# ashispati/ar-vae

Measured on AMD Instinct MI355X. Metric: training images/sec (dSprites beta-VAE+AR, per-GPU batch 512), higher is better.
Workload: dtype f32 (conv MFMAs: scaled 2-term fp16 split, 3 products, fp32-accurate)

## Files before the change

### ar-vae_amd/csrc/conv32.h

```cpp
#pragma once
#include "common.h"
#include "reduce.h"
#include "midprep.h"
#include "regloss.h"

namespace arvae {

bool conv32_fits(const arvae_link_t *l);
int conv32_down(const arvae_link_t *l, const Operand &hi, const float *bias, int relu, const float *gate, const uint16_t *gate_bits,
                uint16_t *bits_out, float *out, hipStream_t s, const float *wprep, const unsigned *amax_in, unsigned *amax_out);
int conv32_up(const arvae_link_t *l, const Operand &lo, const float *bias, int relu, const float *gate, const uint16_t *gate_bits,
              uint16_t *bits_out, float *out, hipStream_t s, const float *wprep, const unsigned *amax_in, unsigned *amax_out);
bool conv32_down_chain_fits(const arvae_link_t *a, const arvae_link_t *b);
int conv32_down_chain(const arvae_link_t *a, const arvae_link_t *b, const float *hi, const unsigned *amax_in, const float *bias_a,
                      uint16_t *bits_a, float *out_a, const float *wprep_a, unsigned *amax_a, const float *bias_b, uint16_t *bits_b,
                      float *out_b, const float *wprep_b, unsigned *amax_b, hipStream_t s);
bool conv32_up_reg_fits(const arvae_link_t *l);
int conv32_up_reg(const arvae_link_t *l, const Operand &lo, const float *bias, uint16_t *bits_out, float *out, const float *wprep,
                  const unsigned *amax_in, unsigned *amax_out, const RegArgs &reg, int r, hipStream_t s);

int64_t conv32_prep_floats();
int64_t conv32_scratch_floats();
int conv32_weight_prep(const float *const *wts, float *const *preps, int n_layers, hipStream_t s);
int conv32_weight_prep_with_mid(const float *const *wts, float *const *preps, int n_layers, const MidPrepArgs &mid, hipStream_t s);
int conv32_amax(const float *x, int64_t count, unsigned *out, hipStream_t s);

int64_t conv32_wgrad_ws_floats(const arvae_link_t *l);
int conv32_wgrad(const arvae_link_t *l, const Operand &lo, const Operand &hi, float *dwt, float *dbias, int bias_mode,
                 float *slab, hipStream_t s, const unsigned *amax_lo, const unsigned *amax_hi);
int conv32_wgrad_partial(const arvae_link_t *l, const Operand &lo, const Operand &hi, float *dwt, float *dbias, int bias_mode,
                         float *slab, hipStream_t s, SlabJob *job, const unsigned *amax_lo, const unsigned *amax_hi);
bool conv32_pair_fits(const arvae_link_t *l, bool up, const float *gate, const uint16_t *gate_bits, int bias_mode);
bool conv32_pair_c1_fits(const arvae_link_t *l, bool up, const uint16_t *gate_bits);
int conv32_pair(const arvae_link_t *l, bool up, const float *g, const float *x_in, const float *gate, const uint16_t *gate_bits,
                float *d_in, const float *wprep, float *dwt, float *dbias, float *slab, hipStream_t s, SlabJob *job,
                const unsigned *amax_g, const unsigned *amax_x, unsigned *amax_out, const float *c1_img, float *c1_slab, SlabJob *c1_job);

}
```

### ar-vae_amd/csrc/conv32.hip

```cpp
#include <mutex>
#include "diag.h"
#include "common.h"
#include "conv32_common.h"
#include "conv32.h"
#include "reduce.h"
#include "midprep.h"
#include "prep32.h"
#include "regloss.h"
#include "down32p.h"
#include "wgrad32r.h"

#include <type_traits>

namespace arvae {

template <int LO, int STRIDE, int PX = 128>
struct PatchLoader {
    using T = Tile<LO, PX>;
    static constexpr int SZ = STRIDE * LO;
    static constexpr int PR = STRIDE * T::TR + 2, PC = STRIDE * T::TC + 2;
    static constexpr int SLOTS = T::TI * PR * PC * 8;
    static constexpr int ITERS = (SLOTS + 255) / 256;
    float4 r[ITERS];
    unsigned rel[ITERS];
// ... 922 lines not shown
            out[16 * C32 * C32 + threadIdx.x] = tot;
        }
    }
}
template <int LO, int BIAS>
__global__ __launch_bounds__(256, 1) void wgrad32x_kernel(const float *__restrict__ lo, const float *__restrict__ hi,
                                                          float *__restrict__ slab, int n_img, int n_tiles, const unsigned *amax_lo,
                                                          const unsigned *amax_hi) {
    wgrad32x_body<LO, BIAS>(lo, hi, slab, n_img, n_tiles, amax_lo, amax_hi, blockIdx.x, gridDim.x);
}

template <int MODE, int BIAS>
__global__ __launch_bounds__(256, 1) void pair4_down_kernel(const float *__restrict__ g_hi, Ep32 ep,
                                                           const float *__restrict__ w_lo, const float *__restrict__ w_hi,
                                                           float *__restrict__ slab, int n_img, int tiles_a, int tiles_b, int grid_a,
                                                           const unsigned *amax_lo, const unsigned *amax_hi) {
    if ((int)blockIdx.x < grid_a) down32s_body<4, MODE>(g_hi, ep, n_img, tiles_a, blockIdx.x, grid_a);
    else wgrad32x_body<4, BIAS>(w_lo, w_hi, slab, n_img, tiles_b, amax_lo, amax_hi, blockIdx.x - grid_a, gridDim.x - grid_a);
}
template <int MODE, int BIAS>
__global__ __launch_bounds__(256, 1) void pair4_up_kernel(const float *__restrict__ g_lo, Ep32 ep,
                                                         const float *__restrict__ w_lo, const float *__restrict__ w_hi,
                                                         float *__restrict__ slab, int n_img, int tiles_a, int tiles_b, int grid_a,
                                                         const unsigned *amax_lo, const unsigned *amax_hi) {
    if ((int)blockIdx.x < grid_a) up32x_body<4, MODE, 32>(g_lo, ep, n_img, tiles_a, blockIdx.x, grid_a);
    else wgrad32x_body<4, BIAS>(w_lo, w_hi, slab, n_img, tiles_b, amax_lo, amax_hi, blockIdx.x - grid_a, gridDim.x - grid_a);
}


template <int LO, int MODE, int BIAS>
__global__ __launch_bounds__(512) __attribute__((amdgpu_waves_per_eu(2, 2))) void pair_down_wgrad_kernel(
    const float *__restrict__ g_hi, Ep32 ep, int n_img, int tiles_a, int grid_a, const float *__restrict__ w_lo, const float *__restrict__ w_hi,
    float *__restrict__ slab, int total_steps, int steps_per_wg, const unsigned *amax_lo, const unsigned *amax_hi) {
    if ((int)blockIdx.x < grid_a) down32p_body<LO, MODE>(g_hi, ep, n_img, tiles_a, blockIdx.x, grid_a);
    else wgrad32r_body<LO, BIAS>(w_lo, w_hi, slab, n_img, total_steps, steps_per_wg, amax_lo, amax_hi, blockIdx.x - grid_a);
}
template <int MODE, int BIAS, bool C1W = false>
__global__ __launch_bounds__(512) __attribute__((amdgpu_waves_per_eu(2, 2))) void pair_up16_wgrad_kernel(
    const float *__restrict__ g_lo, Ep32 ep, int n_img, int tiles_a, int grid_a, const float *__restrict__ w_lo, const float *__restrict__ w_hi,
    float *__restrict__ slab, int total_steps, int steps_per_wg, const unsigned *amax_lo, const unsigned *amax_hi, C1Wgrad c1) {
    if ((int)blockIdx.x < grid_a) up32p_body<MODE, C1W>(g_lo, ep, n_img, tiles_a, blockIdx.x, grid_a, c1);
    else wgrad32r_body<16, BIAS>(w_lo, w_hi, slab, n_img, total_steps, steps_per_wg, amax_lo, amax_hi, blockIdx.x - grid_a);
}
template <int MODE, int BIAS>
__global__ __launch_bounds__(512) __attribute__((amdgpu_waves_per_eu(2, 2))) void pair_up8_wgrad_kernel(
    const float *__restrict__ g_lo, Ep32 ep, int n_img, int tiles_a, int grid_a, const float *__restrict__ w_lo, const float *__restrict__ w_hi,
    float *__restrict__ slab, int total_steps, int steps_per_wg, const unsigned *amax_lo, const unsigned *amax_hi) {
    if ((int)blockIdx.x < grid_a) {
        if (threadIdx.x >= 256) return;
        up32x_body<8, MODE, 32>(g_lo, ep, n_img, tiles_a, blockIdx.x, grid_a);
    } else wgrad32r_body<8, BIAS>(w_lo, w_hi, slab, n_img, total_steps, steps_per_wg, amax_lo, amax_hi, blockIdx.x - grid_a);
}

static int cu_count() { return device_cu_count(); }

template <int LO, int PX = 128> static constexpr int tiles_for(int n) {
    using T = Tile<LO, PX>;
    return T::TI == 1 ? n * (LO / T::TR) : (n + T::TI - 1) / T::TI;
}
static int grid_for_tiles(int tiles) {
    const int cap = cu_count() < AMAX_N / 4 ? cu_count() : AMAX_N / 4;
    return tiles < cap ? tiles : cap;
}

bool conv32_fits(const arvae_link_t *l) {
    return l->chi == 32 && l->clo == 32 && l->kh == 4 && l->kw == 4 && l->stride == 2 && l->pad == 1 &&
           l->hh == l->hw && l->lh == l->lw && (l->lh == 16 || l->lh == 8 || l->lh == 4) && l->hi_perm_c == 0 &&
           l->lo_perm_c == 0 && (int64_t)l->n * l->hh * l->hw * PIXB < (1ll << 31) - (1ll << 20);
}

template <class K> static void allow_lds(K kernel, int bytes) {
    (void)hipFuncSetAttribute((const void *)kernel, hipFuncAttributeMaxDynamicSharedMemorySize, bytes);
}

template <int A, int B> struct MaxOf { static constexpr int value = A > B ? A : B; };

constexpr int LDS_DOWN_S = (PatchLoader<4, 2, 32>::BUF2_DW + 4 * 16 * 64) * 4;
static int down_small_grid(int tiles) {
    int g = tiles < 2 * cu_count() ? tiles : 2 * cu_count();
    return g < AMAX_N ? g : AMAX_N;
}

template <int MODE> static void launch_down_small(const Operand &hi, const Ep32 &ep, int n, hipStream_t s) {
    const int tiles = tiles_for<4, 32>(n);
    static std::once_flag attr;
    std::call_once(attr, [&] { allow_lds(down32s_kernel<4, MODE>, LDS_DOWN_S); });
    ARVAE_LAUNCH((down32s_kernel<4, MODE>), dim3(down_small_grid(tiles)), dim3(256), LDS_DOWN_S, s, hi.v, ep, n, tiles);
}
template <int LO, int MODE, int PX>
static void launch_up_px(const Operand &lo, const Ep32 &ep, int n, hipStream_t s) {
    const int tiles = tiles_for<LO, PX>(n), grid = grid_for_tiles(tiles);
    if constexpr (LO == 16 && PX == 128 && MODE != EP_GATE_F) {
        constexpr int LDSP = (2 * 2 * PatchLoader<16, 1, 128>::PLANE_DW) * 4 + 4 * 4 * 4 * 64 * 16;
        static std::once_flag attrp;
        std::call_once(attrp, [&] { allow_lds(up32p_kernel<MODE>, LDSP); });
        ARVAE_LAUNCH((up32p_kernel<MODE>), dim3(grid), dim3(512), LDSP, s, lo.v, ep, n, tiles);
    } else {
        constexpr int LDSX = 2 * PatchLoader<LO, 1, PX>::PLANE_DW * 4;
        static std::once_flag attrx;
        std::call_once(attrx, [&] { allow_lds(up32x_kernel<LO, MODE, PX>, LDSX); });
        ARVAE_LAUNCH((up32x_kernel<LO, MODE, PX>), dim3(grid), dim3(256), LDSX, s, lo.v, ep, n, tiles);
    }
}
template <int LO, int MODE>
static void launch_up_v(const Operand &lo, const Ep32 &ep, int n, hipStream_t s) {
    if (LO == 4 && 2 * tiles_for<LO, 128>(n) <= cu_count()) launch_up_px<4, MODE, 32>(lo, ep, n, s);
// ... 186 lines not shown
        allow_lds(wgrad32r_kernel<LO, 2>, LDS);
    });
    if (bias_mode == 1) ARVAE_LAUNCH((wgrad32r_kernel<LO, 1>), dim3(grid), dim3(512), LDS, s, lo, hi, slab, l->n, total, spw, amax_lo, amax_hi);
    else if (bias_mode == 2) ARVAE_LAUNCH((wgrad32r_kernel<LO, 2>), dim3(grid), dim3(512), LDS, s, lo, hi, slab, l->n, total, spw, amax_lo, amax_hi);
    else ARVAE_LAUNCH((wgrad32r_kernel<LO, 0>), dim3(grid), dim3(512), LDS, s, lo, hi, slab, l->n, total, spw, amax_lo, amax_hi);
    return check_launch(LO == 16 ? "wgrad32_kernel<16>" : "wgrad32_kernel<8>");
}
static int conv32_wgrad_stream(const arvae_link_t *l, const Operand &lo, const Operand &hi, float *slab, int bias_mode, const unsigned *amax_lo,
                               const unsigned *amax_hi, hipStream_t s) {
    return l->lh == 16 ? launch_stream<16>(l, lo.v, hi.v, slab, bias_mode, amax_lo, amax_hi, s)
                       : launch_stream<8>(l, lo.v, hi.v, slab, bias_mode, amax_lo, amax_hi, s);
}

static int conv32_wgrad_groups(const arvae_link_t *l) {
    if (conv32_wgrad_stream_fits(l)) return conv32_wgrad_stream_groups(l);
    return grid_for_tiles(tiles_for<4, 64>(l->n));
}

int64_t conv32_wgrad_ws_floats(const arvae_link_t *l) {
    return (int64_t)conv32_wgrad_groups(l) * WG32_SLAB;
}

constexpr int LDS_WGRAD_X4 = 2 * (PatchLoader<4, 2, 64>::PLANE_DW / PSB * WGRAD_PSB_H + 64 * WGRAD_PSB_L) * 4;
static int launch_wgrad_x4(const arvae_link_t *l, const Operand &lo, const Operand &hi, float *slab, int bias_mode, int grid,
                           const unsigned *amax_lo, const unsigned *amax_hi, hipStream_t s) {
    const int tiles = tiles_for<4, 64>(l->n);
    static std::once_flag attr;
    std::call_once(attr, [&] {
        allow_lds(wgrad32x_kernel<4, 0>, LDS_WGRAD_X4);
        allow_lds(wgrad32x_kernel<4, 1>, LDS_WGRAD_X4);
        allow_lds(wgrad32x_kernel<4, 2>, LDS_WGRAD_X4);
    });
    if (bias_mode == 1)
        ARVAE_LAUNCH((wgrad32x_kernel<4, 1>), dim3(grid), dim3(256), LDS_WGRAD_X4, s, lo.v, hi.v, slab, l->n, tiles, amax_lo, amax_hi);
    else if (bias_mode == 2)
        ARVAE_LAUNCH((wgrad32x_kernel<4, 2>), dim3(grid), dim3(256), LDS_WGRAD_X4, s, lo.v, hi.v, slab, l->n, tiles, amax_lo, amax_hi);
    else
        ARVAE_LAUNCH((wgrad32x_kernel<4, 0>), dim3(grid), dim3(256), LDS_WGRAD_X4, s, lo.v, hi.v, slab, l->n, tiles, amax_lo, amax_hi);
    return check_launch("wgrad32_kernel<4>");
}

int conv32_wgrad_partial(const arvae_link_t *l, const Operand &lo, const Operand &hi, float *dwt, float *dbias, int bias_mode,
                         float *slab, hipStream_t s, SlabJob *job, const unsigned *amax_lo, const unsigned *amax_hi) {
    ARVAE_REQUIRE(amax_lo != nullptr && amax_hi != nullptr, "conv32_wgrad: the operands' maxima are needed");
    const int grid = conv32_wgrad_groups(l);
    const int rc = conv32_wgrad_stream_fits(l) ? conv32_wgrad_stream(l, lo, hi, slab, bias_mode, amax_lo, amax_hi, s)
                                               : launch_wgrad_x4(l, lo, hi, slab, bias_mode, grid, amax_lo, amax_hi, s);
    *job = SlabJob{slab, dwt, bias_mode ? dbias : nullptr, grid, SLAB_C32, bias_mode};
    return rc;
}

constexpr int PAIR_SPLIT_C1_PERCENT = 62;
constexpr int PAIR_SPLIT_PERCENT = 50;
bool conv32_pair_fits(const arvae_link_t *l, bool up, const float *gate, const uint16_t *gate_bits, int bias_mode) {
    static const bool off4 = diag_env("ARVAE_NO_PAIR4") != nullptr;
    static const bool off = diag_env("ARVAE_NO_PAIR32") != nullptr;
    if ((gate == nullptr && gate_bits == nullptr) || bias_mode != (up ? 2 : 1)) return false;
    if (l->lh == 4) {
        const int wg_tiles = tiles_for<4, 64>(l->n), dg_tiles = tiles_for<4, 32>(l->n);
        return !off4 && wg_tiles >= 8 && wg_tiles + (dg_tiles + 1) / 2 <= cu_count() && conv32_wgrad_groups(l) == wg_tiles;
    }
    if (off || gate_bits == nullptr || !conv32_wgrad_stream_fits(l)) return false;
    if (l->n * (l->lh * l->lh / 32) < 4 * cu_count()) return false;
    if (!up && l->lh == 8 && tiles_for<8, 128>(l->n) > cu_count()) return false;
    return true;
}

template <int LO> static int launch_pair_big(const arvae_link_t *l, bool up, const float *g, const float *x_in, const Ep32 &ep, float *slab,
                                             const unsigned *amax_g, const unsigned *amax_x, hipStream_t s, int *grid_b_out,
                                             const C1Wgrad *c1 = nullptr, int *grid_a_out = nullptr) {
    const int cus = cu_count() < AMAX_N / 4 ? cu_count() : AMAX_N / 4;
    int grid_a = cus * (c1 != nullptr ? PAIR_SPLIT_C1_PERCENT : PAIR_SPLIT_PERCENT) / 100;
    if (grid_a < 1) grid_a = 1;
    const int tiles_a = up ? l->n * DownK<LO>::TILES_PER_IMG : (LO == 16 ? tiles_for<16, 128>(l->n) : tiles_for<8, 32>(l->n));
    {
        const int run = (tiles_a + grid_a - 1) / grid_a;
        grid_a = (tiles_a + run - 1) / run;
    }
    if (grid_a_out != nullptr) *grid_a_out = grid_a;
    ARVAE_REQUIRE(c1 == nullptr || grid_a <= 256, "pair_up16_wgrad: %d workgroups of the Up half exceed the first layer's 256 weight-gradient slabs", grid_a);
    int total, spw, grid_b;
    stream_geometry(l, cus - grid_a, total, spw, grid_b);
    *grid_b_out = grid_b;
    constexpr int LDS_W = RowStream<LO>::LDS_DW * 4;
    const dim3 grid(grid_a + grid_b);
    if (up) {
        constexpr int LDS = MaxOf<LDS_W, DownK<LO>::LDS_DW * 4>::value;
        static std::once_flag attr;
        std::call_once(attr, [&] { allow_lds(pair_down_wgrad_kernel<LO, EP_GATE_B, 2>, LDS); });
        ARVAE_LAUNCH((pair_down_wgrad_kernel<LO, EP_GATE_B, 2>), grid, dim3(512), LDS, s, g, ep, l->n, tiles_a, grid_a, x_in, g, slab, total, spw,
                     amax_x, amax_g);
        return check_launch(LO == 16 ? "pair(down32<16> + wgrad32<16>)" : "pair(down32<8> + wgrad32<8>)");
    }
    if constexpr (LO == 16) {
        constexpr int LDS_U = (2 * 2 * PatchLoader<16, 1, 128>::PLANE_DW) * 4 + 4 * 4 * 4 * 64 * 16;
        constexpr int LDS = MaxOf<LDS_W, LDS_U>::value;
        static std::once_flag attr;
        if (c1 != nullptr) {
            constexpr int LDS_C = MaxOf<LDS_W, LDS_U + 4 * C1W_WAVE_DW * 4>::value;
            static std::once_flag attr_c;
            std::call_once(attr_c, [&] { allow_lds(pair_up16_wgrad_kernel<EP_GATE_B, 1, true>, LDS_C); });
            ARVAE_LAUNCH((pair_up16_wgrad_kernel<EP_GATE_B, 1, true>), grid, dim3(512), LDS_C, s, g, ep, l->n, tiles_a, grid_a, g, x_in,
                         slab, total, spw, amax_g, amax_x, *c1);
            return check_launch("pair(up32<16> + wgrad32<16> + wgrad_c1)");
        }
        std::call_once(attr, [&] { allow_lds(pair_up16_wgrad_kernel<EP_GATE_B, 1>, LDS); });
        ARVAE_LAUNCH((pair_up16_wgrad_kernel<EP_GATE_B, 1>), grid, dim3(512), LDS, s, g, ep, l->n, tiles_a, grid_a, g, x_in, slab,
                     total, spw, amax_g, amax_x, C1Wgrad{nullptr, nullptr});
        return check_launch("pair(up32<16> + wgrad32<16>)");
    } else {
        constexpr int LDS = MaxOf<LDS_W, 2 * PatchLoader<8, 1, 32>::PLANE_DW * 4>::value;
        static std::once_flag attr;
        std::call_once(attr, [&] { allow_lds(pair_up8_wgrad_kernel<EP_GATE_B, 1>, LDS); });
        ARVAE_LAUNCH((pair_up8_wgrad_kernel<EP_GATE_B, 1>), grid, dim3(512), LDS, s, g, ep, l->n, tiles_a, grid_a, g, x_in, slab, total,
                     spw, amax_g, amax_x);
        return check_launch("pair(up32<8> + wgrad32<8>)");
    }
}

bool conv32_pair_c1_fits(const arvae_link_t *l, bool up, const uint16_t *gate_bits) {
    return !up && l->lh == 16 && gate_bits != nullptr;
}
int conv32_pair(const arvae_link_t *l, bool up, const float *g, const float *x_in, const float *gate, const uint16_t *gate_bits,
                float *d_in, const float *wprep, float *dwt, float *dbias, float *slab, hipStream_t s, SlabJob *job,
                const unsigned *amax_g, const unsigned *amax_x, unsigned *amax_out, const float *c1_img, float *c1_slab, SlabJob *c1_job) {
    ARVAE_REQUIRE(wprep != nullptr && amax_g != nullptr && amax_x != nullptr, "conv32_pair: prepared weights and the operands' maxima are needed");
    Ep32 ep{nullptr, gate_bits ? nullptr : gate, gate_bits, nullptr, d_in, reinterpret_cast<const uint4 *>(wprep), amax_g, amax_out};
    if (l->lh != 4) {
        int grid_b = 0, grid_a = 0;
        C1Wgrad c1{c1_img, c1_slab};
        const bool fuse = c1_img != nullptr && c1_slab != nullptr && c1_job != nullptr && conv32_pair_c1_fits(l, up, gate_bits);
        ARVAE_REQUIRE(fuse || c1_img == nullptr, "conv32_pair: this layer cannot carry the first layer's weight gradient");
        const int rc = l->lh == 16 ? launch_pair_big<16>(l, up, g, x_in, ep, slab, amax_g, amax_x, s, &grid_b, fuse ? &c1 : nullptr, &grid_a)
                                   : launch_pair_big<8>(l, up, g, x_in, ep, slab, amax_g, amax_x, s, &grid_b);
        *job = SlabJob{slab, dwt, dbias, grid_b, SLAB_C32, up ? 2 : 1};
        if (fuse) *c1_job = SlabJob{c1_slab, nullptr, nullptr, grid_a, SLAB_C1, 1};
        return rc;
    }
    constexpr int LDS_U = 2 * PatchLoader<4, 1, 32>::PLANE_DW * 4;
    constexpr int LDS = MaxOf<LDS_WGRAD_X4, MaxOf<LDS_DOWN_S, LDS_U>::value>::value;
    const int wg_tiles = tiles_for<4, 64>(l->n), dg_tiles = tiles_for<4, 32>(l->n), grid_a = (dg_tiles + 1) / 2;
    static std::once_flag attr;
    std::call_once(attr, [&] {
        allow_lds(pair4_down_kernel<EP_GATE_F, 2>, LDS);
        allow_lds(pair4_down_kernel<EP_GATE_B, 2>, LDS);
        allow_lds(pair4_up_kernel<EP_GATE_F, 1>, LDS);
        allow_lds(pair4_up_kernel<EP_GATE_B, 1>, LDS);
    });
    const dim3 grid(grid_a + wg_tiles);
    if (up) {
        if (gate_bits) ARVAE_LAUNCH((pair4_down_kernel<EP_GATE_B, 2>), grid, dim3(256), LDS, s, g, ep, x_in, g, slab, l->n, dg_tiles, wg_tiles, grid_a, amax_x, amax_g);
        else ARVAE_LAUNCH((pair4_down_kernel<EP_GATE_F, 2>), grid, dim3(256), LDS, s, g, ep, x_in, g, slab, l->n, dg_tiles, wg_tiles, grid_a, amax_x, amax_g);
    } else {
        if (gate_bits) ARVAE_LAUNCH((pair4_up_kernel<EP_GATE_B, 1>), grid, dim3(256), LDS, s, g, ep, g, x_in, slab, l->n, dg_tiles, wg_tiles, grid_a, amax_g, amax_x);
        else ARVAE_LAUNCH((pair4_up_kernel<EP_GATE_F, 1>), grid, dim3(256), LDS, s, g, ep, g, x_in, slab, l->n, dg_tiles, wg_tiles, grid_a, amax_g, amax_x);
    }
    *job = SlabJob{slab, dwt, dbias, wg_tiles, SLAB_C32, up ? 2 : 1};
    return check_launch(up ? "pair4(down32 + wgrad32)" : "pair4(up32 + wgrad32)");
}

int conv32_wgrad(const arvae_link_t *l, const Operand &lo, const Operand &hi, float *dwt, float *dbias, int bias_mode,
                 float *slab, hipStream_t s, const unsigned *amax_lo, const unsigned *amax_hi) {
    SlabJob job;
    if (int rc = conv32_wgrad_partial(l, lo, hi, dwt, dbias, bias_mode, slab, s, &job, amax_lo, amax_hi)) return rc;
    return slab_reduce(job, s);
}

}

#ifdef ARVAE_STAMPS
extern "C" int arvae_debug_stamps(unsigned long long *out, int count) {
    return (int)hipMemcpyFromSymbol(out, HIP_SYMBOL(arvae::g_stamps), sizeof(unsigned long long) * count);
}
#endif
#ifdef D32K_STAMPS
extern "C" int arvae_debug_d32k_stamps(unsigned long long *out, int count) {
    return (int)hipMemcpyFromSymbol(out, HIP_SYMBOL(arvae::g_d32k_stamps), sizeof(unsigned long long) * count);
}
#endif
#ifdef WGR_STAMPS
extern "C" int arvae_debug_wgr_stamps(unsigned long long *out, int count) {
    return (int)hipMemcpyFromSymbol(out, HIP_SYMBOL(arvae::g_wgr_stamps), sizeof(unsigned long long) * count);
}
#endif
```

### ar-vae_amd/csrc/plan.hip

```cpp
#include "diag.h"
#include "common.h"
#include "dense.h"
#include "reduce.h"
#include "midprep.h"
#include "regloss.h"
#include "vae_finish.h"
#include "amax.h"
#include "conv32.h"
#include "conv_c1.h"
#include "conv64.h"
#include "link.h"
#include "heads.h"
#include "midblock.h"
#include "losses.h"

namespace arvae {

__global__ __launch_bounds__(256) void latent_bwd_full_kernel(const float *__restrict__ g_z, const float *__restrict__ dz_reg,
                                                               const float *__restrict__ dz_extra, const float *__restrict__ mu,
                                                               const float *__restrict__ sigma, const float *__restrict__ eps,
                                                               const float *__restrict__ g_loss, const float *__restrict__ kl,
                                                               const float *__restrict__ cap, float beta, float inv_batch,
                                                               float reg_scale, int64_t count, float *__restrict__ d_mu,
                                                               float *__restrict__ d_ls) {
// ... 214 lines not shown
                if (int rc = conv32_amax(a.in, in_elems(l, a.n), a.tmp_amax, hs)) return rc;
                in_amax = a.tmp_amax;
            }
            return l.is_up ? conv32_up(&lk, make_operand(&op), b, 1, nullptr, nullptr, a.bits_out, a.out, hs, a.wprep, in_amax, a.out_amax)
                           : conv32_down(&lk, make_operand(&op), b, 1, nullptr, nullptr, a.bits_out, a.out, hs, a.wprep, in_amax, a.out_amax);
        }
        return conv_c1_down(&lk, make_operand(&op), w, b, 1, nullptr, nullptr, a.bits_out, a.out, hs, a.out_amax);
    }
    if (conv64_fits(&lk, l.is_up != 0) && a.tmp_amax != nullptr && wide_stack(&lk)) {
        hipStream_t hs = as_stream(a.st);
        if (in_amax == nullptr && conv64s_fits(&lk, l.is_up != 0)) {
            if (int rc = conv32_amax(a.in, in_elems(l, a.n), a.tmp_amax, hs)) return rc;
            in_amax = a.tmp_amax;
        }
        a.out_has = a.out_amax != nullptr;
        return l.is_up ? conv64_up(&lk, make_operand(&op), w, b, l.act, a.mask, a.out, a.link_ws, hs, nullptr, in_amax, a.out_amax, a.wide_prep)
                       : conv64_down(&lk, make_operand(&op), w, b, l.act, a.mask, a.out, a.link_ws, hs, nullptr, in_amax, a.out_amax, a.wide_prep);
    }
    if (!l.is_up && a.out_amax != nullptr && wide_stack(&lk) && !conv64_fits(&lk, false) && single_channel_down_fits(&lk)) {
        a.out_has = true;
        return single_channel_down(&lk, make_operand(&op), w, b, l.act, a.mask, a.out, as_stream(a.st), a.out_amax);
    }
    return l.is_up ? arvae_link_up(&lk, &op, w, b, l.act, a.mask, a.out, a.link_ws, a.st)
                   : arvae_link_down(&lk, &op, w, b, l.act, a.mask, a.out, a.link_ws, a.st);
}

struct LayerBwd {
    const arvae_layer_t *l;
    int32_t n;
    const float *params;
    float *grads;
    const float *in, *out;
    const uint8_t *mask;
    const float *g;
    bool g_is_pre;
    const float *g_scale;
    const float *gate;
    const uint16_t *gate_bits;
    const GateOp *gate_op;
    GateOp gate_store;
    float *d_in;
    float *slab, *link_ws, *own_slab;
    DenseWgradBatch *defer;
    SlabReduceBatch *rdefer;
    arvae_stream_t st;
    const float *wprep;
    float *wide_prep;
    const unsigned *g_amax, *in_amax;
    unsigned *tmp_amax, *tmp2_amax, *din_amax;
    const float *c1_img;
    float *c1_slab;
    SlabJob *c1_job;
    const VaeFinishArgs *finish;
    bool gated;
    bool din_has;
    bool finish_taken;
};

static int layer_backward(LayerBwd &a) {
    const arvae_layer_t &l = *a.l;
    const int32_t n = a.n;
    const arvae_link_t lk = with_batch(l, n);
    const arvae_stream_t st = a.st;
    const float *const g = a.g, *const in = a.in, *const gate = a.gate;
    const uint16_t *const gate_bits = a.gate_bits;
    float *const d_in = a.d_in;
    const unsigned *g_amax = a.g_amax, *in_amax = a.in_amax;
    a.gated = a.din_has = a.finish_taken = false;
    const bool c32 = conv32_fits(&lk) && a.wprep != nullptr && a.tmp_amax != nullptr && a.tmp2_amax != nullptr;
    auto need_g = [&]() -> int {
        if (g_amax != nullptr) return ARVAE_OK;
        g_amax = a.tmp_amax;
        return conv32_amax(g, out_elems(l, n), a.tmp_amax, as_stream(st));
    };
    auto need_in = [&]() -> int {
        if (in_amax != nullptr) return ARVAE_OK;
        in_amax = a.tmp2_amax;
        return conv32_amax(in, in_elems(l, n), a.tmp2_amax, as_stream(st));
    };
    arvae_operand_t gop = a.g_is_pre ? plain(g) : arvae_operand_t{g, a.out, a.mask, l.act};
    if (!a.g_is_pre && (a.mask != nullptr || l.act != ARVAE_ACT_NONE) && (conv64_fits(&lk, false) || conv64_fits(&lk, true))) {
        if (int rc = arvae_operand_apply(&gop, out_elems(l, n), const_cast<float *>(g), st)) return rc;
        gop = plain(g);
        g_amax = nullptr;
    }
    const arvae_operand_t xin = plain(in);
    const float *w = a.params + l.w_off;
    float *dw = a.grads + l.w_off, *db = bias_of(l, a.grads);
    const int bias_mode = db ? (l.is_up ? 2 : 1) : 0;
    hipStream_t hs = as_stream(st);
    const bool own_slab_free = a.rdefer != nullptr && a.own_slab != nullptr && a.rdefer->count < SLAB_BATCH_MAX;
    if (d_in != nullptr && own_slab_free && gop.y == nullptr && a.g_scale == nullptr && c32 &&
        conv32_pair_fits(&lk, l.is_up != 0, gate, gate_bits, bias_mode)) {
        SlabJob job;
        if (int rc = need_g()) return rc;
        if (int rc = need_in()) return rc;
        const bool c1 = a.c1_img != nullptr && a.c1_slab != nullptr && a.c1_job != nullptr && conv32_pair_c1_fits(&lk, l.is_up != 0, gate_bits);
        if (int rc = conv32_pair(&lk, l.is_up != 0, gop.v, in, gate, gate_bits, d_in, a.wprep, dw, db, a.own_slab, hs, &job, g_amax, in_amax,
                                  c1 ? nullptr : a.din_amax, c1 ? a.c1_img : nullptr, c1 ? a.c1_slab : nullptr, c1 ? a.c1_job : nullptr))
            return rc;
        slab_reduce_defer(a.rdefer, job);
        a.gated = true;
        a.din_has = !c1 && a.din_amax != nullptr;
        return ARVAE_OK;
    }
    const bool simple = gop.mask == nullptr && gop.act != ARVAE_ACT_SELU;
    if (d_in != nullptr && l.is_up && gate != nullptr && simple && gop.y == nullptr && own_slab_free && conv_c1_pair_fits(&lk)) {
        Operand g_op = make_operand(&gop);
        g_op.scale = a.g_scale;
        SlabJob job;
        if (int rc = conv_c1_pair(&lk, g_op, w, gate_bits ? nullptr : gate, gate_bits, d_in, make_operand(&xin), dw, db, bias_mode, a.own_slab,
                                  hs, &job, a.din_amax, a.finish))
            return rc;
        a.finish_taken = a.finish != nullptr;
        slab_reduce_defer(a.rdefer, job);
        a.gated = true;
        a.din_has = a.din_amax != nullptr;
        return ARVAE_OK;
    }
    if (d_in != nullptr) {
        int rc;
        if (l.is_up) {
            if (gate != nullptr && gop.y == nullptr && c32) {
                if (int rc2 = need_g()) return rc2;
                rc = conv32_down(&lk, make_operand(&gop), nullptr, 0, gate_bits ? nullptr : gate, gate_bits, nullptr, d_in, hs, a.wprep,
                                 g_amax, a.din_amax);
                a.gated = true;
                a.din_has = a.din_amax != nullptr;
            } else if (gate != nullptr && simple && conv_c1_fits(&lk)) {
                Operand g_op = make_operand(&gop);
                g_op.scale = a.g_scale;
                rc = conv_c1_down(&lk, g_op, w, nullptr, 0, gate_bits ? nullptr : gate, gate_bits, nullptr, d_in, hs, a.din_amax);
                a.gated = true;
                a.din_has = a.din_amax != nullptr;
            } else if (a.gate_op != nullptr && !conv64_fits(&lk, false) && !conv_c1_fits(&lk) && single_channel_down_gated_fits(&lk)) {
                rc = single_channel_down_gated(&lk, make_operand(&gop), w, a.gate_op, d_in, hs, a.din_amax);
                a.gated = true;
                a.din_has = a.din_amax != nullptr && lk.n <= 1024;
            } else if (a.gate_op != nullptr && conv64s_fits(&lk, false)) {
                if (gop.y == nullptr && a.tmp_amax != nullptr)
                    if (int rc2 = need_g()) return rc2;
                rc = conv64_down(&lk, make_operand(&gop), w, nullptr, ARVAE_ACT_NONE, nullptr, d_in, a.link_ws, hs, a.gate_op,
                                 gop.y == nullptr ? g_amax : nullptr, a.din_amax, a.wide_prep);
                a.gated = true;
                a.din_has = a.din_amax != nullptr;
            } else {
                rc = arvae_link_down(&lk, &gop, w, nullptr, ARVAE_ACT_NONE, nullptr, d_in, a.link_ws, st);
            }
        } else {
            if (gate != nullptr && gop.y == nullptr && c32) {
                if (int rc2 = need_g()) return rc2;
                rc = conv32_up(&lk, make_operand(&gop), nullptr, 0, gate_bits ? nullptr : gate, gate_bits, nullptr, d_in, hs, a.wprep,
                               g_amax, a.din_amax);
                a.gated = true;
// ... 350 lines not shown
        if (producer.act == ARVAE_ACT_RELU && mask_of(mask_idx) == nullptr) return nullptr;
        go.y = saved; go.mask = mask_of(mask_idx); go.act = producer.act;
        return &go;
    };
    bool pre = true;
    auto common_args = [&](LayerBwd &a, const arvae_layer_t &l, const float *in, const float *g, float *d_in) {
        a = LayerBwd{};
        a.l = &l; a.n = batch; a.params = params; a.grads = grads; a.in = in; a.g = g; a.g_is_pre = true; a.d_in = d_in;
        a.slab = V.slab; a.link_ws = V.link_ws; a.defer = &defer; a.st = stream;
    };
    auto layer_args = [&](LayerBwd &a, bool dec, int i, float *dst) {
        const arvae_layer_t *layers = dec ? m->dec : m->enc;
        const LayerBufs *B = dec ? V.dec : V.enc;
        const int *mask_idx = dec ? dec_mask : enc_mask;
        const arvae_layer_t &l = layers[i];
        common_args(a, l, i > 0 ? B[i - 1].out : (dec ? z : x), cur, dst);
        a.out = (dec && i + 1 == m->n_dec) ? logits : B[i].out;
        a.mask = mask_of(mask_idx[i]);
        a.g_is_pre = pre;
        a.g_amax = cur_amax;
        if (i > 0) {
            a.gate = relu_gate(layers[i - 1], mask_idx[i - 1], a.in);
            a.gate_op = general_gate(layers[i - 1], mask_idx[i - 1], a.in, a.gate_store);
            a.gate_bits = a.gate != nullptr ? B[i - 1].bits : nullptr;
            const arvae_link_t lk = with_batch(l, batch);
            const bool fast = B[i].bits != nullptr && B[i].wprep != nullptr;
            if (fast || (conv64s_fits(&lk, l.is_up != 0) && wide_stack(&lk))) a.in_amax = B[i - 1].amax;
        }
        a.own_slab = B[i].slab;
        a.rdefer = &rdefer;
        a.wprep = B[i].wprep;
        a.wide_prep = B[i].wide[l.is_up ? 0 : 1];
        a.tmp_amax = V.tmp_amax; a.tmp2_amax = V.tmp2_amax; a.din_amax = grad_amax(dst);
    };
    {
        const int li = m->n_dec - 1;
        const arvae_layer_t &last = m->dec[li];
        const arvae_link_t lk = with_batch(last, batch);
        const bool fold = last.is_up && conv_c1_fits(&lk) && mask_of(dec_mask[li]) == nullptr && li > 0 &&
                          relu_gate(m->dec[li - 1], dec_mask[li - 1], V.dec[li - 1].out) != nullptr && V.dec[li].slab != nullptr;
        if (fold) {
            cur = V.dlogits;
            first_scale = g_loss;
        } else {
            cur = grad_dst(V.dec[li].keep, nullptr);
            if (int rc = arvae_scale_by_scalar(g_loss, V.dlogits, pix, cur, stream)) return rc;
        }
    }
    int mid_ne = 0, mid_nd = 0;
    const bool mid = mid_fusable(m, &mid_ne, &mid_nd);
    const bool fold = mid && fold_conv_layers(m, L, batch, masks, mid_ne, mid_nd);
    bool finish_pending = finish_deferred(m);
    const float *heads_next_g = nullptr;
    for (int i = m->n_dec - 1; i >= (mid ? mid_nd + (fold ? 1 : 0) : 0); --i) {
        float *dst = grad_dst(i > 0 ? V.dec[i - 1].keep : nullptr, cur);
        if (i == 0 && !mid && pre && m->n_dec > 1 && heads_fusable(&m->head_mu, &m->head_log_std, m->zdim) &&
            heads_next_fusable(&m->dec[0], m->zdim) && mask_of(dec_mask[0]) == nullptr) {
            heads_next_g = cur;
            dst = nullptr;
        }
        const bool carry = finish_pending && i == m->n_dec - 1;
        LayerBwd a;
        layer_args(a, true, i, dst);
        a.g_scale = i == m->n_dec - 1 ? first_scale : nullptr;
        a.finish = carry ? V.fin_args : nullptr;
        if (int rc = layer_backward(a)) return rc;
        if (carry) {
            if (!a.finish_taken)
                if (int rc = vae_finish_deferred(V.fin_args, st)) return rc;
            finish_pending = false;
        }
        pre = a.gated;
        if (heads_next_g == nullptr) { cur = dst; cur_amax = a.din_has ? grad_amax(dst) : nullptr; }
    }
    const arvae_milestones *ms = m->milestones;
    bool dec_marked = false, lin_marked = false;
    if (ms != nullptr && ms->dec_grads != nullptr && defer.count == 0) {
        if (int rc = slab_reduce_flush(&rdefer, st)) return rc;
        mark(ms->dec_grads, st);
        dec_marked = true;
    }
    const float *hidden = V.enc[m->n_enc - 1].out;
    const float *dz_reg = (reg_fused == 1 && m->n_reg > 0) ? V.dz_reg : reg_fused == 2 ? dz_extra : nullptr;
    if (reg_fused == 2) {
        ARVAE_REQUIRE(dz_extra != nullptr, "image_vae_backward: reg_fused 2 needs the unit regulariser gradient in dz_extra");
        dz_extra = nullptr;
    }
    const float *kl = V.kld_out + 1;
    const float *head_gate = relu_gate(m->enc[m->n_enc - 1], enc_mask[m->n_enc - 1], hidden);
    float *d_hidden = V.enc[m->n_enc - 1].keep;
    auto queue_wgrad = [&](const arvae_layer_t &l, const float *g, const float *in) -> int {
        const arvae_link_t lk = with_batch(l, batch);
        float *dw = grads + l.w_off, *db = bias_of(l, grads);
        const arvae_operand_t gop = plain(g), xin = plain(in);
        if (dense_wgrad_defer(&defer, &lk, make_operand(&gop), in, dw, db)) return ARVAE_OK;
        return arvae_link_wgrad(&lk, &gop, &xin, dw, db, db ? 1 : 0, V.slab, stream);
    };
    int enc_from = m->n_enc - 1;
    if (mid) {
        const int e0 = m->n_enc - mid_ne;
        float *enc_y[ARVAE_MAX_LAYERS], *dec_y[ARVAE_MAX_LAYERS], *enc_g[ARVAE_MAX_LAYERS], *dec_g[ARVAE_MAX_LAYERS];
        for (int i = 0; i < mid_ne; ++i) { enc_y[i] = V.enc[e0 + i].out; enc_g[i] = V.enc[e0 + i].keep; }
        for (int i = 0; i < mid_nd; ++i) { dec_y[i] = V.dec[i].out; dec_g[i] = V.dec[i].keep; }
        const float *x0 = V.enc[e0 - 1].out;
        const float *gate0 = relu_gate(m->enc[e0 - 1], enc_mask[e0 - 1], x0);
        float *d_x0 = V.enc[e0 - 1].keep;
        const float *g_last = cur;
        MidFold mf{};
        if (fold) {
            ARVAE_REQUIRE(pre, "image_vae_backward: the folded conv layer needs a gated upstream gradient");
            mf.hi_e = V.enc[e0 - 2].out;
            mf.g_hi_d = cur;
// ... 38 lines not shown
            lin_marked = true;
        }
    } else if (heads_fusable(&m->head_mu, &m->head_log_std, m->zdim)) {
        if (int rc = heads_latent_bwd(&m->head_mu, &m->head_log_std, batch, m->zdim, params, heads_next_g != nullptr ? nullptr : cur,
                                      dz_reg, dz_extra, mu, sigma, eps, g_loss, kl, capacity, m->beta, reg_scale,
                                      head_gate, V.d_mu, V.d_ls, d_hidden, st,
                                      heads_next_g != nullptr ? &m->dec[0] : nullptr, heads_next_g))
            return rc;
        if (int rc = queue_wgrad(m->head_mu, V.d_mu, hidden)) return rc;
        if (int rc = queue_wgrad(m->head_log_std, V.d_ls, hidden)) return rc;
        cur = d_hidden;
        cur_amax = nullptr;
        pre = head_gate != nullptr;
    } else {
        int64_t blocks = (bz + 255) / 256;
        if (blocks > 1024) blocks = 1024;
        ARVAE_LAUNCH(latent_bwd_full_kernel, dim3((unsigned)blocks), dim3(256), 0, st, cur, dz_reg, dz_extra, mu, sigma,
                           eps, g_loss, kl, capacity, m->beta, 1.f / (float)batch, reg_scale, bz,
                           V.d_mu, V.d_ls);
        if (int rc = check_launch("image_vae_backward(latent)")) return rc;
        cur = d_hidden;
        float *other = grad_dst(nullptr, cur);
        LayerBwd a;
        common_args(a, m->head_mu, hidden, V.d_mu, cur);
        if (int rc = layer_backward(a)) return rc;
        common_args(a, m->head_log_std, hidden, V.d_ls, other);
        if (int rc = layer_backward(a)) return rc;
        const int64_t hn = in_elems(m->head_mu, batch);
        int64_t blocks2 = (hn + 255) / 256;
        if (blocks2 > 2048) blocks2 = 2048;
        ARVAE_LAUNCH(add_inplace_kernel, dim3((unsigned)blocks2), dim3(256), 0, st, cur, other, head_gate, hn);
        if (int rc = check_launch("image_vae_backward(add)")) return rc;
        pre = head_gate != nullptr;
        cur_amax = nullptr;
    }
    SlabJob c1_job{};
    bool c1_possible = false;
    if (enc_from >= 1 && masks == nullptr && V.enc[0].slab != nullptr && V.enc[0].bits != nullptr) {
        const arvae_link_t lk0 = with_batch(m->enc[0], batch);
        c1_possible = !m->enc[0].is_up && m->enc[0].act == ARVAE_ACT_RELU && m->enc[0].dropout == 0 && conv_c1_fits(&lk0) && lk0.hh == 64 &&
                      lk0.hw == 64 && lk0.clo == 32 && m->enc[0].b_off >= 0;
    }
    for (int i = enc_from; i >= 0; --i) {
        if (i == 0 && c1_job.slab != nullptr) {
            c1_job.dwt = grads + m->enc[0].w_off;
            c1_job.dbias = grads + m->enc[0].b_off;
            ARVAE_REQUIRE(slab_reduce_defer(&rdefer, c1_job), "image_vae_backward: too many slab reductions queued");
            break;
        }
        float *dst = i > 0 ? grad_dst(V.enc[i - 1].keep, cur) : nullptr;
        LayerBwd a;
        layer_args(a, false, i, dst);
        if (i == 1 && c1_possible) { a.c1_img = x; a.c1_slab = V.enc[0].slab; a.c1_job = &c1_job; }
        if (int rc = layer_backward(a)) return rc;
        pre = a.gated;
        cur = dst;
        cur_amax = a.din_has ? grad_amax(dst) : nullptr;
    }
    if (int rc = dense_wgrad_slab_flush(&defer, &rdefer, st)) return rc;
    if (ms != nullptr) {
        if (!dec_marked) mark(ms->dec_grads, st);
        if (!lin_marked) mark(ms->linear_grads, st);
    }
    return ARVAE_OK;
}
```

Before: 1.455 million.

## Chain two decoder backward data-grad convs and defer second wgrad into encoder pair

Adds a fused kernel that runs the backward data-gradient of two consecutive 32-channel decoder up-convs (16x16 then 8x8) in one launch, alongside the first layer's weight-gradient on the remaining CUs. The second layer's weight-gradient is deferred and carried as an extra wgrad job inside the encoder's 8x8 pair launch, with a fallback standalone wgrad if no carrier appears. The aim is fewer launches and better CU filling in the small-spatial layers. In exchange it adds intricate planning logic, grid split heuristics and LDS sizing, and the fused path only applies when tile counts divide evenly.

```diff
diff --git a/ar-vae_amd/csrc/conv32.h b/ar-vae_amd/csrc/conv32.h
--- a/ar-vae_amd/csrc/conv32.h
+++ b/ar-vae_amd/csrc/conv32.h
@@ -30,10 +30,23 @@
                  float *slab, hipStream_t s, const unsigned *amax_lo, const unsigned *amax_hi);
 int conv32_wgrad_partial(const arvae_link_t *l, const Operand &lo, const Operand &hi, float *dwt, float *dbias, int bias_mode,
                          float *slab, hipStream_t s, SlabJob *job, const unsigned *amax_lo, const unsigned *amax_hi);
+struct WgradRide {
+    const float *lo, *hi;
+    const unsigned *amax_lo, *amax_hi;
+    float *slab, *dwt, *dbias;
+    int n;
+};
 bool conv32_pair_fits(const arvae_link_t *l, bool up, const float *gate, const uint16_t *gate_bits, int bias_mode);
 bool conv32_pair_c1_fits(const arvae_link_t *l, bool up, const uint16_t *gate_bits);
+bool conv32_pair_ride_fits(const arvae_link_t *l, bool up, const WgradRide *ride);
 int conv32_pair(const arvae_link_t *l, bool up, const float *g, const float *x_in, const float *gate, const uint16_t *gate_bits,
                 float *d_in, const float *wprep, float *dwt, float *dbias, float *slab, hipStream_t s, SlabJob *job,
-                const unsigned *amax_g, const unsigned *amax_x, unsigned *amax_out, const float *c1_img, float *c1_slab, SlabJob *c1_job);
+                const unsigned *amax_g, const unsigned *amax_x, unsigned *amax_out, const float *c1_img, float *c1_slab, SlabJob *c1_job,
+                const WgradRide *ride = nullptr, SlabJob *ride_job = nullptr);
+bool conv32_pair_chain_fits(const arvae_link_t *a, const arvae_link_t *b, const uint16_t *gate_bits_a, const uint16_t *gate_bits_b);
+int conv32_pair_chain(const arvae_link_t *a, const arvae_link_t *b, const float *g, const float *x_in_a, const uint16_t *gate_bits_a,
+                      float *d_in_a, const float *wprep_a, float *dwt_a, float *dbias_a, float *slab_a, const unsigned *amax_g,
+                      const unsigned *amax_x_a, unsigned *amax_out_a, const uint16_t *gate_bits_b, float *d_in_b, const float *wprep_b,
+                      unsigned *amax_out_b, hipStream_t s, SlabJob *job_a);
 
 }
diff --git a/ar-vae_amd/csrc/conv32.hip b/ar-vae_amd/csrc/conv32.hip
--- a/ar-vae_amd/csrc/conv32.hip
+++ b/ar-vae_amd/csrc/conv32.hip
@@ -998,6 +998,37 @@
     } else wgrad32r_body<8, BIAS>(w_lo, w_hi, slab, n_img, total_steps, steps_per_wg, amax_lo, amax_hi, blockIdx.x - grid_a);
 }
 
+__global__ __launch_bounds__(512) __attribute__((amdgpu_waves_per_eu(2, 2))) void pair_chain_down_wgrad_kernel(
+    const float *__restrict__ g_hi, Ep32 ep_a, Ep32 ep_b, int n_img, int tiles_a, int tiles_b, int grid_a, const float *__restrict__ w_lo,
+    const float *__restrict__ w_hi, float *__restrict__ slab, int total_steps, int steps_per_wg, const unsigned *amax_lo, const unsigned *amax_hi) {
+    if ((int)blockIdx.x < grid_a) {
+        extern __shared__ __attribute__((aligned(16))) unsigned chain_lds[];
+        constexpr int BODY_DW = DownK<16>::LDS_DW > DownK<8>::LDS_DW ? DownK<16>::LDS_DW : DownK<8>::LDS_DW;
+        float *chain_max = reinterpret_cast<float *>(chain_lds + BODY_DW);
+        down32p_body<16, EP_GATE_B, 1>(g_hi, ep_a, n_img, tiles_a, blockIdx.x, grid_a, chain_max);
+        __syncthreads();
+        down32p_body<8, EP_GATE_B, 2>(ep_a.out, ep_b, n_img, tiles_b, blockIdx.x, grid_a, chain_max);
+    } else wgrad32r_body<16, 2>(w_lo, w_hi, slab, n_img, total_steps, steps_per_wg, amax_lo, amax_hi, blockIdx.x - grid_a);
+}
+struct WgradJob8 {
+    const float *lo, *hi;
+    float *slab;
+    const unsigned *amax_lo, *amax_hi;
+    int total_steps, steps_per_wg, grid;
+};
+template <int MODE>
+__global__ __launch_bounds__(512) __attribute__((amdgpu_waves_per_eu(2, 2))) void pair_up8_wgrad2_kernel(
+    const float *__restrict__ g_lo, Ep32 ep, int n_img, int tiles_a, int grid_a, WgradJob8 first, WgradJob8 second) {
+    if ((int)blockIdx.x < grid_a) {
+        if (threadIdx.x >= 256) return;
+        up32x_body<8, MODE, 32>(g_lo, ep, n_img, tiles_a, blockIdx.x, grid_a);
+        return;
+    }
+    const int w = blockIdx.x - grid_a;
+    if (w < first.grid) wgrad32r_body<8, 1>(first.lo, first.hi, first.slab, n_img, first.total_steps, first.steps_per_wg, first.amax_lo, first.amax_hi, w);
+    else wgrad32r_body<8, 2>(second.lo, second.hi, second.slab, n_img, second.total_steps, second.steps_per_wg, second.amax_lo, second.amax_hi, w - first.grid);
+}
+
 static int cu_count() { return device_cu_count(); }
 
 template <int LO, int PX = 128> static constexpr int tiles_for(int n) {
@@ -1290,6 +1321,13 @@
 
 constexpr int PAIR_SPLIT_C1_PERCENT = 62;
 constexpr int PAIR_SPLIT_PERCENT = 50;
+#ifndef ARVAE_PAIR_SPLIT_CHAIN
+#define ARVAE_PAIR_SPLIT_CHAIN 50
+#endif
+#ifndef ARVAE_PAIR_SPLIT_UP8_TWO
+#define ARVAE_PAIR_SPLIT_UP8_TWO 38
+#endif
+constexpr int PAIR_SPLIT_CHAIN_PERCENT = ARVAE_PAIR_SPLIT_CHAIN, PAIR_SPLIT_UP8_TWO_PERCENT = ARVAE_PAIR_SPLIT_UP8_TWO;
 bool conv32_pair_fits(const arvae_link_t *l, bool up, const float *gate, const uint16_t *gate_bits, int bias_mode) {
     static const bool off4 = diag_env("ARVAE_NO_PAIR4") != nullptr;
     static const bool off = diag_env("ARVAE_NO_PAIR32") != nullptr;
@@ -1359,11 +1397,48 @@
 bool conv32_pair_c1_fits(const arvae_link_t *l, bool up, const uint16_t *gate_bits) {
     return !up && l->lh == 16 && gate_bits != nullptr;
 }
+static int launch_pair_up8_two(const arvae_link_t *l, const float *g, const float *x_in, const Ep32 &ep, float *slab, const unsigned *amax_g,
+                               const unsigned *amax_x, const WgradRide &ride, hipStream_t s, int *grid_b_out, int *grid_r_out) {
+    const int cus = cu_count() < AMAX_N / 4 ? cu_count() : AMAX_N / 4;
+    int grid_a = cus * PAIR_SPLIT_UP8_TWO_PERCENT / 100;
+    if (grid_a < 1) grid_a = 1;
+    const int tiles_a = tiles_for<8, 32>(l->n);
+    {
+        const int run = (tiles_a + grid_a - 1) / grid_a;
+        grid_a = (tiles_a + run - 1) / run;
+    }
+    const int rest = cus - grid_a > 2 ? cus - grid_a : 2;
+    WgradJob8 first{g, x_in, slab, amax_g, amax_x, 0, 0, 0}, second{ride.lo, ride.hi, ride.slab, ride.amax_lo, ride.amax_hi, 0, 0, 0};
+    stream_geometry(l, rest / 2, first.total_steps, first.steps_per_wg, first.grid);
+    stream_geometry(l, rest - rest / 2, second.total_steps, second.steps_per_wg, second.grid);
+    *grid_b_out = first.grid;
+    *grid_r_out = second.grid;
+    constexpr int LDS = MaxOf<RowStream<8>::LDS_DW * 4, 2 * PatchLoader<8, 1, 32>::PLANE_DW * 4>::value;
+    static std::once_flag attr;
+    std::call_once(attr, [&] { allow_lds(pair_up8_wgrad2_kernel<EP_GATE_B>, LDS); });
+    ARVAE_LAUNCH((pair_up8_wgrad2_kernel<EP_GATE_B>), dim3(grid_a + first.grid + second.grid), dim3(512), LDS, s, g, ep, l->n, tiles_a, grid_a,
+                 first, second);
+    return check_launch("pair(up32<8> + wgrad32<8> + wgrad32<8>)");
+}
+bool conv32_pair_ride_fits(const arvae_link_t *l, bool up, const WgradRide *ride) {
+    return ride != nullptr && !up && l->lh == 8 && ride->n == l->n && ride->lo != nullptr && ride->hi != nullptr && ride->slab != nullptr &&
+           ride->amax_lo != nullptr && ride->amax_hi != nullptr;
+}
+
 int conv32_pair(const arvae_link_t *l, bool up, const float *g, const float *x_in, const float *gate, const uint16_t *gate_bits,
                 float *d_in, const float *wprep, float *dwt, float *dbias, float *slab, hipStream_t s, SlabJob *job,
-                const unsigned *amax_g, const unsigned *amax_x, unsigned *amax_out, const float *c1_img, float *c1_slab, SlabJob *c1_job) {
+                const unsigned *amax_g, const unsigned *amax_x, unsigned *amax_out, const float *c1_img, float *c1_slab, SlabJob *c1_job,
+                const WgradRide *ride, SlabJob *ride_job) {
     ARVAE_REQUIRE(wprep != nullptr && amax_g != nullptr && amax_x != nullptr, "conv32_pair: prepared weights and the operands' maxima are needed");
     Ep32 ep{nullptr, gate_bits ? nullptr : gate, gate_bits, nullptr, d_in, reinterpret_cast<const uint4 *>(wprep), amax_g, amax_out};
+    if (ride != nullptr) {
+        ARVAE_REQUIRE(ride_job != nullptr && gate_bits != nullptr && conv32_pair_ride_fits(l, up, ride), "conv32_pair: this launch cannot carry the second weight-gradient job");
+        int grid_b = 0, grid_r = 0;
+        const int rc = launch_pair_up8_two(l, g, x_in, ep, slab, amax_g, amax_x, *ride, s, &grid_b, &grid_r);
+        *job = SlabJob{slab, dwt, dbias, grid_b, SLAB_C32, 1};
+        *ride_job = SlabJob{ride->slab, ride->dwt, ride->dbias, grid_r, SLAB_C32, 2};
+        return rc;
+    }
     if (l->lh != 4) {
         int grid_b = 0, grid_a = 0;
         C1Wgrad c1{c1_img, c1_slab};
@@ -1397,6 +1472,43 @@
     return check_launch(up ? "pair4(down32 + wgrad32)" : "pair4(up32 + wgrad32)");
 }
 
+static int pair_chain_grid(const arvae_link_t *a, const arvae_link_t *b) {
+    const int cus = cu_count() < AMAX_N / 4 ? cu_count() : AMAX_N / 4;
+    if (a->n != b->n || a->n < cus) return 0;
+    int target = cus * PAIR_SPLIT_CHAIN_PERCENT / 100;
+    if (target < 1) target = 1;
+    const int ipw = (a->n + target - 1) / target, grid = (a->n + ipw - 1) / ipw;
+    const int tiles_a = a->n * DownK<16>::TILES_PER_IMG, tiles_b = b->n * DownK<8>::TILES_PER_IMG;
+    const int run_a = (tiles_a + grid - 1) / grid, run_b = (tiles_b + grid - 1) / grid;
+    return (grid < cus && run_a * DownK<8>::TILES_PER_IMG == run_b * DownK<16>::TILES_PER_IMG) ? grid : 0;
+}
+bool conv32_pair_chain_fits(const arvae_link_t *a, const arvae_link_t *b, const uint16_t *gate_bits_a, const uint16_t *gate_bits_b) {
+    static const bool off = diag_env("ARVAE_NO_BWD_CHAIN") != nullptr;
+    return !off && gate_bits_b != nullptr && conv32_fits(a) && conv32_fits(b) && a->lh == 16 && b->lh == 8 && b->hh == a->lh &&
+           conv32_pair_fits(a, true, nullptr, gate_bits_a, 2) && pair_chain_grid(a, b) > 0;
+}
+int conv32_pair_chain(const arvae_link_t *a, const arvae_link_t *b, const float *g, const float *x_in_a, const uint16_t *gate_bits_a,
+                      float *d_in_a, const float *wprep_a, float *dwt_a, float *dbias_a, float *slab_a, const unsigned *amax_g,
+                      const unsigned *amax_x_a, unsigned *amax_out_a, const uint16_t *gate_bits_b, float *d_in_b, const float *wprep_b,
+                      unsigned *amax_out_b, hipStream_t s, SlabJob *job_a) {
+    ARVAE_REQUIRE(conv32_pair_chain_fits(a, b, gate_bits_a, gate_bits_b), "conv32_pair_chain: these two layers do not chain");
+    ARVAE_REQUIRE(g && x_in_a && d_in_a && d_in_b && wprep_a && wprep_b && slab_a && amax_g && amax_x_a && amax_out_a && job_a,
+                  "conv32_pair_chain: null pointer");
+    Ep32 ep_a{nullptr, nullptr, gate_bits_a, nullptr, d_in_a, reinterpret_cast<const uint4 *>(wprep_a), amax_g, amax_out_a};
+    Ep32 ep_b{nullptr, nullptr, gate_bits_b, nullptr, d_in_b, reinterpret_cast<const uint4 *>(wprep_b), nullptr, amax_out_b};
+    const int cus = cu_count() < AMAX_N / 4 ? cu_count() : AMAX_N / 4;
+    const int grid_a = pair_chain_grid(a, b);
+    int total, spw, grid_b;
+    stream_geometry(a, cus - grid_a, total, spw, grid_b);
+    constexpr int LDS = MaxOf<RowStream<16>::LDS_DW * 4, (MaxOf<DownK<16>::LDS_DW, DownK<8>::LDS_DW>::value + 4) * 4>::value;
+    static std::once_flag attr;
+    std::call_once(attr, [&] { allow_lds(pair_chain_down_wgrad_kernel, LDS); });
+    ARVAE_LAUNCH(pair_chain_down_wgrad_kernel, dim3(grid_a + grid_b), dim3(512), LDS, s, g, ep_a, ep_b, a->n, a->n * DownK<16>::TILES_PER_IMG,
+                 b->n * DownK<8>::TILES_PER_IMG, grid_a, x_in_a, g, slab_a, total, spw, amax_x_a, amax_g);
+    *job_a = SlabJob{slab_a, dwt_a, dbias_a, grid_b, SLAB_C32, 2};
+    return check_launch("chain(down32<16> + down32<8>) + wgrad32<16>");
+}
+
 int conv32_wgrad(const arvae_link_t *l, const Operand &lo, const Operand &hi, float *dwt, float *dbias, int bias_mode,
                  float *slab, hipStream_t s, const unsigned *amax_lo, const unsigned *amax_hi) {
     SlabJob job;
diff --git a/ar-vae_amd/csrc/plan.hip b/ar-vae_amd/csrc/plan.hip
--- a/ar-vae_amd/csrc/plan.hip
+++ b/ar-vae_amd/csrc/plan.hip
@@ -290,9 +290,11 @@
     float *c1_slab;
     SlabJob *c1_job;
     const VaeFinishArgs *finish;
+    const WgradRide *ride;
     bool gated;
     bool din_has;
     bool finish_taken;
+    bool ride_taken;
 };
 
 static int layer_backward(LayerBwd &a) {
@@ -304,7 +306,7 @@
     const uint16_t *const gate_bits = a.gate_bits;
     float *const d_in = a.d_in;
     const unsigned *g_amax = a.g_amax, *in_amax = a.in_amax;
-    a.gated = a.din_has = a.finish_taken = false;
+    a.gated = a.din_has = a.finish_taken = a.ride_taken = false;
     const bool c32 = conv32_fits(&lk) && a.wprep != nullptr && a.tmp_amax != nullptr && a.tmp2_amax != nullptr;
     auto need_g = [&]() -> int {
         if (g_amax != nullptr) return ARVAE_OK;
@@ -334,10 +336,17 @@
         if (int rc = need_g()) return rc;
         if (int rc = need_in()) return rc;
         const bool c1 = a.c1_img != nullptr && a.c1_slab != nullptr && a.c1_job != nullptr && conv32_pair_c1_fits(&lk, l.is_up != 0, gate_bits);
+        const bool ride = !c1 && gate_bits != nullptr && a.rdefer->count + 1 < SLAB_BATCH_MAX && conv32_pair_ride_fits(&lk, l.is_up != 0, a.ride);
+        SlabJob ride_job;
         if (int rc = conv32_pair(&lk, l.is_up != 0, gop.v, in, gate, gate_bits, d_in, a.wprep, dw, db, a.own_slab, hs, &job, g_amax, in_amax,
-                                  c1 ? nullptr : a.din_amax, c1 ? a.c1_img : nullptr, c1 ? a.c1_slab : nullptr, c1 ? a.c1_job : nullptr))
+                                  c1 ? nullptr : a.din_amax, c1 ? a.c1_img : nullptr, c1 ? a.c1_slab : nullptr, c1 ? a.c1_job : nullptr,
+                                  ride ? a.ride : nullptr, ride ? &ride_job : nullptr))
             return rc;
         slab_reduce_defer(a.rdefer, job);
+        if (ride) {
+            slab_reduce_defer(a.rdefer, ride_job);
+            a.ride_taken = true;
+        }
         a.gated = true;
         a.din_has = !c1 && a.din_amax != nullptr;
         return ARVAE_OK;
@@ -794,12 +803,44 @@
     const bool fold = mid && fold_conv_layers(m, L, batch, masks, mid_ne, mid_nd);
     bool finish_pending = finish_deferred(m);
     const float *heads_next_g = nullptr;
-    for (int i = m->n_dec - 1; i >= (mid ? mid_nd + (fold ? 1 : 0) : 0); --i) {
+    const int dec_from = mid ? mid_nd + (fold ? 1 : 0) : 0;
+    const arvae_milestones *ms0 = m->milestones;
+    WgradRide ride{};
+    const arvae_layer_t *ride_layer = nullptr;
+    bool ride_pending = false;
+    for (int i = m->n_dec - 1; i >= dec_from; --i) {
         float *dst = grad_dst(i > 0 ? V.dec[i - 1].keep : nullptr, cur);
         if (i == 0 && !mid && pre && m->n_dec > 1 && heads_fusable(&m->head_mu, &m->head_log_std, m->zdim) &&
             heads_next_fusable(&m->dec[0], m->zdim) && mask_of(dec_mask[0]) == nullptr) {
             heads_next_g = cur;
             dst = nullptr;
+        }
+        if (i >= 2 && i - 1 >= dec_from && i < m->n_dec - 1 && dst != nullptr && pre && cur_amax != nullptr &&
+            V.dec[i - 1].keep != nullptr && V.dec[i - 2].keep != nullptr &&
+            !(ms0 != nullptr && ms0->dec_grads != nullptr) && rdefer.count + 2 <= SLAB_BATCH_MAX) {
+            float *dst_b = grad_dst(V.dec[i - 2].keep, dst);
+            LayerBwd a, b;
+            layer_args(a, true, i, dst);
+            layer_args(b, true, i - 1, dst_b);
+            const arvae_link_t lka = with_batch(*a.l, batch), lkb = with_batch(*b.l, batch);
+            float *db_a = bias_of(*a.l, grads), *db_b = bias_of(*b.l, grads);
+            if (a.l->is_up && b.l->is_up && a.gate_bits != nullptr && b.gate_bits != nullptr && a.wprep != nullptr && b.wprep != nullptr &&
+                a.in_amax != nullptr && b.in_amax != nullptr && a.din_amax != nullptr && a.own_slab != nullptr && b.own_slab != nullptr &&
+                db_a != nullptr && db_b != nullptr && conv32_pair_chain_fits(&lka, &lkb, a.gate_bits, b.gate_bits)) {
+                SlabJob job;
+                if (int rc = conv32_pair_chain(&lka, &lkb, cur, a.in, a.gate_bits, dst, a.wprep, grads + a.l->w_off, db_a, a.own_slab, cur_amax,
+                                               a.in_amax, a.din_amax, b.gate_bits, dst_b, b.wprep, b.din_amax, st, &job))
+                    return rc;
+                slab_reduce_defer(&rdefer, job);
+                ride = WgradRide{b.in, dst, b.in_amax, a.din_amax, b.own_slab, grads + b.l->w_off, db_b, batch};
+                ride_layer = b.l;
+                ride_pending = true;
+                --i;
+                pre = true;
+                cur = dst_b;
+                cur_amax = b.din_amax;
+                continue;
+            }
         }
         const bool carry = finish_pending && i == m->n_dec - 1;
         LayerBwd a;
@@ -944,10 +985,22 @@
         LayerBwd a;
         layer_args(a, false, i, dst);
         if (i == 1 && c1_possible) { a.c1_img = x; a.c1_slab = V.enc[0].slab; a.c1_job = &c1_job; }
+        a.ride = ride_pending ? &ride : nullptr;
         if (int rc = layer_backward(a)) return rc;
+        if (a.ride_taken) ride_pending = false;
         pre = a.gated;
         cur = dst;
         cur_amax = a.din_has ? grad_amax(dst) : nullptr;
+    }
+    if (ride_pending) {
+        const arvae_link_t lkr = with_batch(*ride_layer, batch);
+        const arvae_operand_t rlo = plain(ride.lo), rhi = plain(ride.hi);
+        SlabJob job;
+        if (int rc = conv32_wgrad_partial(&lkr, make_operand(&rlo), make_operand(&rhi), ride.dwt, ride.dbias, 2, ride.slab, st, &job,
+                                          ride.amax_lo, ride.amax_hi))
+            return rc;
+        if (!slab_reduce_defer(&rdefer, job))
+            if (int rc = slab_reduce(job, st)) return rc;
     }
     if (int rc = dense_wgrad_slab_flush(&defer, &rdefer, st)) return rc;
     if (ms != nullptr) {
```

New measurement: 1.470 million (median of 5 runs). 1.0% higher.
